# tum-vision/dvo_slam

Hardware: AMD Instinct MI355X
Metric: frame-pair alignments/s (640x480, 4-level pyramid) + finest-level HBM GB/s vs roofline (higher is better)
Workload: dtype f32 (Gram operands exact f16 hi + lo pairs on every level, f32 accumulate); 1 GPU; 1024 pairs (BASELINE config 4): independent 640x480 RGB-D frame pairs, seeds 0..1023, pair i on rank i mod 1, 4-level pyramid, FirstLevel=3, LastLevel=0, MaxIterationsPerLevel=100, Precision=5e-7, Mu=0; step = every rank re-ingests the raw planes of its shard from HBM (pyramids, sampling planes, point selection) and aligns it as one batch; the build of step k+1 (build stream) overlaps the match of; pairs=1024, pairs_per_gpu=1024, width=640, height=480, lanes=1 lane

## Files before the change

dvo_slam_amd/csrc/capi.hip:

```cpp
#include <hip/hip_runtime.h>
#ifdef DVO_WITH_ROCTX
#include <rocprofiler-sdk-roctx/roctx.h>
#endif
#include <xmmintrin.h>

#include <algorithm>
#include <functional>
#include <climits>
#include <cstddef>
#include <cmath>
#include <cstdio>
#include <atomic>
#include <chrono>
#include <thread>
#include <condition_variable>
#include <cstdlib>
#include <cstring>
#include <mutex>
#include <string>
#include <vector>

#include "../../include/dvo_hip.h"
#include "device_types.h"
#include "batch_policy.h"
#include "colour.h"
#include "launch.h"
#include "pose_graph.h"
#include "ref_order.h"
#include "selection.h"

using namespace dvo_hip;

namespace {

std::string g_create_error;

std::atomic<unsigned long long> g_free_epoch{1};

struct DevBuf {
  void* p = nullptr;
  size_t bytes = 0;
  hipError_t reserve(size_t n) {
    if (n <= bytes) return hipSuccess;
    if (p) {
      (void)hipFree(p);
      g_free_epoch.fetch_add(1, std::memory_order_relaxed);
    }
    p = nullptr;
    bytes = 0;
    hipError_t e = hipMalloc(&p, n);
    if (e == hipSuccess) bytes = n;
    return e;
  }
  void release() {
    if (p) {
      (void)hipFree(p);
      g_free_epoch.fetch_add(1, std::memory_order_relaxed);
    }
    p = nullptr;
    bytes = 0;
  }
  template <typename T> T* as() const { return static_cast<T*>(p); }
};

struct PinnedBuf {
  void* p = nullptr;
  size_t bytes = 0;
  hipError_t reserve(size_t n) {
    if (n <= bytes) return hipSuccess;
    release();
    hipError_t e = hipHostMalloc(&p, n, hipHostMallocCoherent | hipHostMallocMapped);
    if (e == hipSuccess) bytes = n;
    else p = nullptr;
    return e;
  }
  void release() {
    if (p) (void)hipHostFree(p);
    p = nullptr;
    bytes = 0;
  }
  template <typename T> T* as() const { return static_cast<T*>(p); }
};

struct CameraGeom {
  int w0 = 0, h0 = 0, levels = 0;
  float K0[4] = {0, 0, 0, 0};
  int w[kMaxLevels], h[kMaxLevels];
  float K[kMaxLevels][4];
  float* tx[kMaxLevels];
  float* ty[kMaxLevels];
  DevBuf tables;
};

struct FrameLevel {
  int w = 0, h = 0;
  float* I = nullptr;
  float* Z = nullptr;
  float4* A = nullptr;
  float2* B = nullptr;
  float2* R = nullptr;
  float2* C = nullptr;
  int cur_have = 0;
  bool selected = false;
  bool q3 = false;
  bool explicit_sel = false;
  float ithr = 0, dthr = 0;
};
// ... 201 lines not shown
  int cap_levels = 0, cap_iters = 0;
  hipEvent_t after = nullptr;
  int rc = DVO_HIP_OK;
};


struct dvo_hip_context {
  std::recursive_mutex mutex;
  int device = 0;
  hipStream_t stream = nullptr;
  std::string err;
  int opt_rows_per_wave = 0;
  int opt_iters_per_sync = 0;
  struct MatchRequest {
    dvo_hip_frame* reference; dvo_hip_frame* current; const dvo_hip_config* cfg; dvo_hip_result* result;
    dvo_hip_level_stats* levels; int cap_levels; dvo_hip_iteration_stats* iters; int cap_iters;
    std::atomic<int> state{0};
    int rc = 0;
  };
  std::mutex rendezvous_mutex;
  MatchRequest* rendezvous_waiting = nullptr;
  dvo_hip_frame* rendezvous_busy_current = nullptr;
  int rendezvous_expect = 0;
  int opt_rendezvous = 1;
  long long rendezvous_pairs = 0;
  long long f16_range_repeats = 0;
  long long strip_ingests = 0;
  long long colour_ingests = 0;
  long long f32_ingests = 0;
  long long lens_ingests = 0;
  long long depth_registrations = 0;
  long long map_inserts = 0, map_points = 0, map_dropped = 0;
  long long map_removes = 0, map_rehashes = 0;
  int opt_graph_resident = 0;
  long long graph_resident_solves = 0;
  long long map_renders = 0;
  struct DeferredIngest {
    std::vector<dvo_hip_frame*> frames;
    std::vector<const void*> planes, depth;
    int format = 0;
    size_t pitch = 0;
    int depth_format = 0;
    size_t depth_pitch = 0;
    float depth_scale;
    int role;
    dvo_hip_config cfg;
    bool keep_raw_copy;
  };
  std::vector<DeferredIngest> deferred;
  int opt_defer_ingest = 0;
  int opt_defer_ingest_pixels = 0;
  int opt_keep_raw_copy = 1;
  long long deferred_ingests = 0;
  int opt_build_workgroups = 0;
  int opt_stream_policy = 1;
  int opt_tail_speculation = 0;
  int opt_solver_waves = 0;
  int opt_ll_blocks = 0;
  int opt_compact_residuals = 1;
  int opt_gram_lo_parts = 1;
  int opt_min_workgroups = 0;
  int opt_condition_number = 0;
  int opt_fused_ll_pixels = 0;
  float last_sel_ithr = 0.0f, last_sel_dthr = 0.0f;
  int f32_gram_hold = 0;
  long long warmup_wait_us = 0;
  int opt_variant = 8;
  int opt_resident = -1;
  int opt_resident_rows = 0;
  int opt_resident_group = 0;
  int resident_timeouts = 0;
  long long resident_launches = 0;
  long long resident_levels = 0;
  long long host_ns[4] = {0, 0, 0, 0};
  long long host_batches = 0;
  std::chrono::steady_clock::time_point batch_entry;
  int opt_resident_flags = 0;
  int opt_sweep_tail = 0;
  long long tail_steps = 0;
  int opt_overlap_tails = 0;
  int opt_overlap_fraction = 8;
  int opt_tail_lists = 0;
  long long listed_steps = 0;
  long long overlapped_tails = 0;
  long long overlapped_steps = 0;
  long long tail_drains = 0;
  long long tail_wait_ns = 0;
  int opt_batch_groups = 0;
  bool is_twin = false;
  std::vector<GroupWorker*> group_workers;
  hipEvent_t roles_ready = nullptr;
  long long grouped_batches = 0;
  int opt_small_sweep = 0;
  int opt_small_tiles = 0;
  int opt_coarse = 0;
  int opt_coarse_pixels = 0;
  int opt_coarse_wgs = 0;
  long long coarse_launches = 0, coarse_levels = 0;
  int opt_deterministic = 0;
  int opt_ref_compat = 0;
  int opt_ref_order = 0;
  long long ref_order_passes = 0;
  DevBuf ref_order_planes;
  DevBuf rcp_table;
  int rcp_shift = 0;
  int rcp_packed = 0;
  int opt_resident_cooperative = 0;
  int compute_units = 0;
  std::vector<CameraGeom*> cameras;
  struct PooledBlock { void* p; size_t bytes; };
  std::vector<PooledBlock> frame_pool;
  size_t frame_pool_bytes = 0;
  static constexpr size_t kFramePoolMaxBytes = size_t(1) << 30;
  static constexpr size_t kFramePoolMaxBlocks = 64;
  Workspace ws[1];
  DevBuf misc, role_tbl_cur, role_tbl_ref, prep_tbl_cur, prep_tbl_ref;
  DevBuf sel_tbl_main, sel_tbl_build;
  unsigned long long sel_visits = 0;
  DevBuf lens_tbl;
  DevBuf graph_jobs, graph_outs;
  DevBuf rig_tbl;
  DevBuf colour_tbl, colour_stage;
  DevBuf map_tbl, map_stage;
  DevBuf render_tbl, render_zbuf, render_planes;
  hipEvent_t render_done = nullptr;
  static const int kTableSlots = 4;
  DevBuf build_tbl[kTableSlots];
  DevBuf* build_tbl_cur = nullptr;
  unsigned build_tbl_next = 0;
  PinnedRing tables;
  std::vector<dvo_hip_frame*> build_tbl_frames;
  hipStream_t build_stream = nullptr;
  static const int kBuildRing = 16;
  hipEvent_t build_events[kBuildRing] = {};
  unsigned long long build_seq = 0;
  unsigned long long main_waited_seq = 0;
  hipStream_t upload_stream = nullptr;
  hipEvent_t upload_done = nullptr;
  static const int kUploadRing = 3;
  DevBuf upload_buf[kUploadRing];
  unsigned long long upload_buf_seq[kUploadRing] = {};
  unsigned upload_next = 0;
  unsigned long long upload_waited_seq = 0;
};

namespace {
int flush_deferred(dvo_hip_context* ctx);
}

#define DVO_FLUSH_DEFERRED(ctx)                                     \
  do {                                                              \
    if ((ctx) && !(ctx)->deferred.empty()) {                        \
      const int rc_deferred__ = flush_deferred(ctx);                \
      if (rc_deferred__ != DVO_HIP_OK) return rc_deferred__;        \
    }                                                               \
  } while (0)

#define DVO_LOCK(ctx)                                               \
  std::unique_lock<std::recursive_mutex> guard;                     \
  if (ctx) guard = std::unique_lock<std::recursive_mutex>((ctx)->mutex)
#define DVO_ENTER(ctx) \
  DVO_LOCK(ctx);       \
  DVO_FLUSH_DEFERRED(ctx)

namespace {

// ... 914 lines not shown
```

dvo_slam_amd/csrc/capi_groups.inc:

```
void mirror_options(const dvo_hip_context* from, dvo_hip_context* to) {
#define DVO_MIRROR(f) to->f = from->f
  DVO_MIRROR(opt_rows_per_wave); DVO_MIRROR(opt_iters_per_sync); DVO_MIRROR(opt_tail_speculation); DVO_MIRROR(opt_solver_waves);
  DVO_MIRROR(opt_ll_blocks); DVO_MIRROR(opt_compact_residuals); DVO_MIRROR(opt_gram_lo_parts); DVO_MIRROR(opt_min_workgroups);
  DVO_MIRROR(opt_condition_number); DVO_MIRROR(opt_fused_ll_pixels); DVO_MIRROR(opt_variant); DVO_MIRROR(opt_resident);
  DVO_MIRROR(opt_resident_rows); DVO_MIRROR(opt_resident_group); DVO_MIRROR(opt_resident_flags); DVO_MIRROR(opt_resident_cooperative);
  DVO_MIRROR(opt_sweep_tail); DVO_MIRROR(opt_coarse); DVO_MIRROR(opt_coarse_pixels); DVO_MIRROR(opt_coarse_wgs);
  DVO_MIRROR(opt_deterministic); DVO_MIRROR(opt_ref_order); DVO_MIRROR(opt_small_sweep); DVO_MIRROR(opt_small_tiles); DVO_MIRROR(compute_units);
  DVO_MIRROR(opt_overlap_tails); DVO_MIRROR(opt_overlap_fraction); DVO_MIRROR(opt_tail_lists); DVO_MIRROR(opt_defer_ingest_pixels);
#undef DVO_MIRROR
}

void group_worker_main(GroupWorker* gw) {
  (void)hipSetDevice(gw->twin->device);
  for (;;) {
    std::unique_lock<std::mutex> lock(gw->m);
    gw->cv.wait(lock, [&] { return gw->has_job || gw->quit; });
    if (gw->quit) return;
    gw->has_job = false;
    lock.unlock();
    dvo_hip_context* t = gw->twin;
    t->batch_entry = std::chrono::steady_clock::now();
    int rc = DVO_HIP_OK;
    if (hipStreamWaitEvent(t->stream, gw->after, 0) != hipSuccess) {
      t->err = "match: a pair group could not wait for the batch's role planes";
      rc = DVO_HIP_ERR_HIP;
    }
    if (rc == DVO_HIP_OK) {
      rc = run_batch(t, gw->n, gw->refs, gw->curs, gw->cfg, gw->results, gw->levels, gw->cap_levels, gw->iters, gw->cap_iters);
      if (rc != DVO_HIP_OK) t->err = t->ws[0].err;
    }
    lock.lock();
    gw->rc = rc;
    gw->done = true;
    lock.unlock();
    gw->cv.notify_all();
  }
}

int batch_groups_of(const dvo_hip_context* ctx, int n) {
  if (ctx->is_twin || ctx->opt_ref_compat || ctx->opt_deterministic || ctx->opt_ref_order) return 1;
  return ctx->opt_batch_groups > 1 ? std::min(ctx->opt_batch_groups, std::max(1, n / 64)) : 1;
}

int ensure_group_workers(dvo_hip_context* ctx, int groups) {
  while (int(ctx->group_workers.size()) < groups - 1) {
    dvo_hip_context* twin = nullptr;
    const int rc = dvo_hip_context_create(ctx->device, &twin);
    if (rc != DVO_HIP_OK) return fail(ctx, rc, "match: could not create a pair group's context");
    twin->is_twin = true;
    GroupWorker* gw = new GroupWorker();
    gw->twin = twin;
    gw->thread = std::thread(group_worker_main, gw);
    ctx->group_workers.push_back(gw);
  }
  if (!ctx->roles_ready) DVO_HIP_TRY(ctx, hipEventCreateWithFlags(&ctx->roles_ready, hipEventDisableTiming));
  return DVO_HIP_OK;
}

void destroy_group_workers(dvo_hip_context* ctx) {
  for (GroupWorker* gw : ctx->group_workers) {
    {
      std::lock_guard<std::mutex> lock(gw->m);
      gw->quit = true;
    }
    gw->cv.notify_all();
    if (gw->thread.joinable()) gw->thread.join();
    dvo_hip_context_destroy(gw->twin);
    delete gw;
  }
  ctx->group_workers.clear();
  if (ctx->roles_ready) (void)hipEventDestroy(ctx->roles_ready);
  ctx->roles_ready = nullptr;
}

int run_batch_grouped(dvo_hip_context* ctx, int groups, int n, dvo_hip_frame* const* refs, dvo_hip_frame* const* curs, const dvo_hip_config* cfg,
                      dvo_hip_result* results, dvo_hip_level_stats* levels, int cap_levels, dvo_hip_iteration_stats* iters, int cap_iters) {
  int rc = ensure_group_workers(ctx, groups);
  if (rc != DVO_HIP_OK) return rc;
  DVO_HIP_TRY(ctx, hipEventRecord(ctx->roles_ready, ctx->stream));
  const int base = n / groups, extra = n % groups;
  const int n0 = base + (extra > 0 ? 1 : 0);
  int at = n0;
  for (int g = 1; g < groups; ++g) {
    GroupWorker* gw = ctx->group_workers[g - 1];
    const int m = base + (g < extra ? 1 : 0);
    mirror_options(ctx, gw->twin);
    {
      std::lock_guard<std::mutex> lock(gw->m);
      gw->n = m;
      gw->refs = refs + at; gw->curs = curs + at; gw->cfg = cfg; gw->results = results + at;
      gw->levels = levels && cap_levels > 0 ? levels + size_t(at) * cap_levels : nullptr;
// ... 27 lines not shown
```

dvo_slam_amd/csrc/capi_options.inc:

```
int dvo_hip_get_counter(dvo_hip_context* ctx, const char* key, long long* value) {
  if (!ctx || !key || !value) return DVO_HIP_ERR_INVALID;
  std::unique_lock<std::recursive_mutex> guard(ctx->mutex);
  if (std::strcmp(key, "resident_launches") == 0) *value = ctx->resident_launches;
  else if (std::strcmp(key, "resident_levels") == 0) *value = ctx->resident_levels;
  else if (std::strcmp(key, "resident_timeouts") == 0) *value = ctx->resident_timeouts;
  else if (std::strcmp(key, "grouped_batches") == 0) *value = ctx->grouped_batches;
  else if (std::strcmp(key, "compute_units") == 0) *value = BatchPolicy(ctx->compute_units).cus;
  else if (std::strcmp(key, "defer_ingest_max_pairs") == 0) *value = BatchPolicy(ctx->compute_units).defer_ingest_max_pairs();
  else if (std::strcmp(key, "background_build_workgroups") == 0) *value = BatchPolicy(ctx->compute_units).background_build_workgroups();
  else if (std::strcmp(key, "tail_steps") == 0) {
    *value = ctx->tail_steps;
    for (const GroupWorker* gw : ctx->group_workers) *value += gw->twin->tail_steps;
  }
  else if (std::strcmp(key, "overlapped_tails") == 0) *value = ctx->overlapped_tails;
  else if (std::strcmp(key, "overlapped_steps") == 0) *value = ctx->overlapped_steps;
  else if (std::strcmp(key, "listed_steps") == 0) *value = ctx->listed_steps;
  else if (std::strcmp(key, "tail_drains") == 0) *value = ctx->tail_drains;
  else if (std::strcmp(key, "tail_wait_us") == 0) *value = ctx->tail_wait_ns / 1000;
  else if (std::strcmp(key, "ref_order_passes") == 0) *value = ctx->ref_order_passes;
  else if (std::strcmp(key, "coarse_launches") == 0) *value = ctx->coarse_launches;
  else if (std::strcmp(key, "coarse_levels") == 0) *value = ctx->coarse_levels;
  else if (std::strcmp(key, "window_fallbacks") == 0) {
    unsigned long long v = 0;
    if (ctx->ws[0].win_fallbacks.p) {
      DVO_HIP_TRY(ctx, hipStreamSynchronize(ctx->stream));
      DVO_HIP_TRY(ctx, hipMemcpy(&v, ctx->ws[0].win_fallbacks.p, sizeof(v), hipMemcpyDeviceToHost));
    }
    *value = (long long)v;
  }
  else if (std::strcmp(key, "strip_ingests") == 0) *value = ctx->strip_ingests;
  else if (std::strcmp(key, "colour_ingests") == 0) *value = ctx->colour_ingests;
  else if (std::strcmp(key, "f32_ingests") == 0) *value = ctx->f32_ingests;
  else if (std::strcmp(key, "lens_ingests") == 0) *value = ctx->lens_ingests;
  else if (std::strcmp(key, "depth_registrations") == 0) *value = ctx->depth_registrations;
  else if (std::strcmp(key, "depth_rig_table_bytes") == 0) *value = (long long)ctx->rig_tbl.bytes;
  else if (std::strcmp(key, "map_inserts") == 0) *value = ctx->map_inserts;
  else if (std::strcmp(key, "map_removes") == 0) *value = ctx->map_removes;
  else if (std::strcmp(key, "map_rehashes") == 0) *value = ctx->map_rehashes;
  else if (std::strcmp(key, "map_renders") == 0) *value = ctx->map_renders;
  else if (std::strcmp(key, "map_points") == 0) *value = ctx->map_points;
  else if (std::strcmp(key, "map_dropped") == 0) *value = ctx->map_dropped;
  else if (std::strcmp(key, "graph_resident_solves") == 0) *value = ctx->graph_resident_solves;
  else if (std::strcmp(key, "warmup_wait_us") == 0) *value = ctx->warmup_wait_us;
  else if (std::strcmp(key, "rendezvous_pairs") == 0) {
    std::lock_guard<std::mutex> lock(ctx->rendezvous_mutex);
    *value = ctx->rendezvous_pairs;
  }
  else if (std::strcmp(key, "f16_range_repeats") == 0) *value = ctx->f16_range_repeats;
  else if (std::strcmp(key, "table_uploads_skipped") == 0) *value = ctx->tables.skipped;
  else if (std::strcmp(key, "deferred_ingests") == 0) *value = ctx->deferred_ingests;
  else if (std::strcmp(key, "host_batches") == 0) *value = ctx->host_batches;
  else if (std::strcmp(key, "host_ns_prepare") == 0) *value = ctx->host_ns[0];
  else if (std::strcmp(key, "host_ns_enqueue") == 0) *value = ctx->host_ns[1];
  else if (std::strcmp(key, "host_ns_wait") == 0) *value = ctx->host_ns[2];
  else if (std::strcmp(key, "host_ns_finish") == 0) *value = ctx->host_ns[3];
  else return fail(ctx, DVO_HIP_ERR_INVALID, "unknown counter");
  return DVO_HIP_OK;
}

int dvo_hip_set_option(dvo_hip_context* ctx, const char* key, int value) {
  DVO_LOCK(ctx);
  if (!ctx || !key) return DVO_HIP_ERR_INVALID;
  if (std::strcmp(key, "rows_per_wave") == 0) {
    if (value != 0 && value != 1 && value != 2 && value != 4 && value != 8 && value != 16)
      return fail(ctx, DVO_HIP_ERR_INVALID, "rows_per_wave must be 0,1,2,4,8,16");
    ctx->opt_rows_per_wave = value;
    return DVO_HIP_OK;
  }
  if (std::strcmp(key, "iters_per_sync") == 0) {
    if (value < 0) return fail(ctx, DVO_HIP_ERR_INVALID, "iters_per_sync must be >= 0");
    ctx->opt_iters_per_sync = value;
    return DVO_HIP_OK;
  }
  if (std::strcmp(key, "variant") == 0) {
    if (value != 0 && (value < 5 || value > 9))
      return fail(ctx, DVO_HIP_ERR_INVALID, "variant must be 0 (all-VALU schedule), 5 (matrix-core schedule), 6 or 7 (current-frame window staged in LDS, residuals bit-identical to the oracle's), 8 or 9 (the same with contracted arithmetic)");
    if (ctx->opt_ref_order && value != 7 && value != 8) return fail(ctx, DVO_HIP_ERR_INVALID, "ref_order runs under variant 7 or 8");
    ctx->opt_variant = value;
    ctx->f32_gram_hold = 0;
    return DVO_HIP_OK;
  }
  if (std::strcmp(key, "rendezvous") == 0) {
    if (value != 0 && value != 1) return fail(ctx, DVO_HIP_ERR_INVALID, "rendezvous must be 0 or 1");
    ctx->opt_rendezvous = value;
    return DVO_HIP_OK;
  }
  if (std::strcmp(key, "ref_order") == 0) {
    if (value != 0 && value != 1) return fail(ctx, DVO_HIP_ERR_INVALID, "ref_order must be 0 or 1");
    if (value && ctx->opt_variant != 7 && ctx->opt_variant != 8) return fail(ctx, DVO_HIP_ERR_INVALID, "ref_order runs under variant 7 or 8");
    ctx->opt_ref_order = value;
    return DVO_HIP_OK;
  }
  if (std::strcmp(key, "deterministic") == 0) {
    if (value != 0 && value != 1) return fail(ctx, DVO_HIP_ERR_INVALID, "deterministic must be 0 or 1");
    ctx->opt_deterministic = value;
    return DVO_HIP_OK;
  }
  if (std::strcmp(key, "ref_compat") == 0) {
    if (value < 0 || value > 2) return fail(ctx, DVO_HIP_ERR_INVALID, "ref_compat must be 0, 1 or 2 (2: as 1, the table read through memory by every sweep)");
    if (value && !ctx->rcp_table.p) {
      const int rc = build_rcp_table(ctx);
      if (rc != DVO_HIP_OK) return rc;
    }
    ctx->opt_ref_compat = value;
    return DVO_HIP_OK;
  }
  if (std::strcmp(key, "resident") == 0) {
    if (value < -1 || value > 1) return fail(ctx, DVO_HIP_ERR_INVALID, "resident must be -1 (automatic), 0 (off) or 1 (every level)");
    ctx->opt_resident = value;
    return DVO_HIP_OK;
  }
  if (std::strcmp(key, "small_sweep") == 0) {
    if (value != 0 && value != 1) return fail(ctx, DVO_HIP_ERR_INVALID, "small_sweep must be 0 or 1");
    ctx->opt_small_sweep = value;
    return DVO_HIP_OK;
  }
  if (std::strcmp(key, "small_tiles") == 0) {
    if (value < 0 || value > 32) return fail(ctx, DVO_HIP_ERR_INVALID, "small_tiles must be 0 (by batch size) .. 32");
    ctx->opt_small_tiles = value;
    return DVO_HIP_OK;
  }
  if (std::strcmp(key, "batch_groups") == 0) {
    if (value < 0 || value > 4) return fail(ctx, DVO_HIP_ERR_INVALID, "batch_groups must be 0 or 1 (one group) .. 4");
    ctx->opt_batch_groups = value;
    return DVO_HIP_OK;
  }
  if (std::strcmp(key, "solver_occupancy") == 0) {
    if (value != 0 && value != 3) return fail(ctx, DVO_HIP_ERR_INVALID, "solver_occupancy must be 0 or 3");
    g_solver_occupancy = value;
    return DVO_HIP_OK;
  }
  if (std::strcmp(key, "sweep_tail") == 0) {
    if (value < 0 || value > 2) return fail(ctx, DVO_HIP_ERR_INVALID, "sweep_tail must be 0, 1 (the whole step in the sweep's tail) or 2 (its wide half; the serial half in a launch behind it)");
    ctx->opt_sweep_tail = value;
    return DVO_HIP_OK;
  }
  if (std::strcmp(key, "overlap_tails") == 0) {
    if (value < 0 || value > 1) return fail(ctx, DVO_HIP_ERR_INVALID, "overlap_tails must be 0 (off) or 1 (a level's stragglers finish beside the next level)");
    ctx->opt_overlap_tails = value;
    return DVO_HIP_OK;
  }
  if (std::strcmp(key, "defer_ingest_pixels") == 0) {
    if (value < 0) return fail(ctx, DVO_HIP_ERR_INVALID, "defer_ingest_pixels must be >= 0");
    ctx->opt_defer_ingest_pixels = value;
    return DVO_HIP_OK;
  }
  if (std::strcmp(key, "tail_lists") == 0) {
    if (value < 0 || value > 1) return fail(ctx, DVO_HIP_ERR_INVALID, "tail_lists must be 0 or 1 (the last steps of a costly level are launched over the list of pairs still on it)");
    ctx->opt_tail_lists = value;
    return DVO_HIP_OK;
  }
  if (std::strcmp(key, "overlap_fraction") == 0) {
    if (value < 2 || value > 64) return fail(ctx, DVO_HIP_ERR_INVALID, "overlap_fraction must be in [2, 64]: a level's tail is split off once at most 1/value of the pairs is on it");
    ctx->opt_overlap_fraction = value;
    return DVO_HIP_OK;
  }
  if (std::strcmp(key, "coarse") == 0) {
    if (value < 0 || value > 1) return fail(ctx, DVO_HIP_ERR_INVALID, "coarse must be 0 (off) or 1 (whenever the levels admit it)");
    ctx->opt_coarse = value;
    return DVO_HIP_OK;
  }
  if (std::strcmp(key, "coarse_pixels") == 0) {
    if (value < 0) return fail(ctx, DVO_HIP_ERR_INVALID, "coarse_pixels must be >= 0");
    ctx->opt_coarse_pixels = value;
    return DVO_HIP_OK;
  }
  if (std::strcmp(key, "coarse_workgroups") == 0) {
    if (value != 0 && value != 3 && value != 4) return fail(ctx, DVO_HIP_ERR_INVALID, "coarse_workgroups must be 0, 3 or 4");
    ctx->opt_coarse_wgs = value;
    return DVO_HIP_OK;
  }
  if (std::strcmp(key, "resident_flags") == 0) {
    ctx->opt_resident_flags = value;
    return DVO_HIP_OK;
  }
  if (std::strcmp(key, "resident_cooperative") == 0) {
    ctx->opt_resident_cooperative = value != 0;
    return DVO_HIP_OK;
  }
  if (std::strcmp(key, "resident_rows") == 0) {
    if (value < 0) return fail(ctx, DVO_HIP_ERR_INVALID, "resident_rows must be >= 0");
    ctx->opt_resident_rows = value;
    return DVO_HIP_OK;
  }
  if (std::strcmp(key, "resident_group") == 0) {
    if (value < 0 || value > kResidentMaxGroup || (value & (value - 1))) return fail(ctx, DVO_HIP_ERR_INVALID, "resident_group must be 0 or a power of two <= 64");
    ctx->opt_resident_group = value;
    return DVO_HIP_OK;
  }
  if (std::strcmp(key, "build_workgroups") == 0) {
    if (value < 0) return fail(ctx, DVO_HIP_ERR_INVALID, "build_workgroups must be >= 0");
    ctx->opt_build_workgroups = value;
    return DVO_HIP_OK;
  }
  if (std::strcmp(key, "tail_speculation") == 0) {
    if (value < 0) return fail(ctx, DVO_HIP_ERR_INVALID, "tail_speculation must be >= 0");
    ctx->opt_tail_speculation = value;
    return DVO_HIP_OK;
  }
  if (std::strcmp(key, "solver_waves") == 0) {
    if (value != 0 && value != 2 && value != 4) return fail(ctx, DVO_HIP_ERR_INVALID, "solver_waves must be 0, 2 or 4");
    ctx->opt_solver_waves = value;
    return DVO_HIP_OK;
  }
  if (std::strcmp(key, "ll_blocks") == 0) {
    if (value < 0 || value > kLlBlocksPerPair) return fail(ctx, DVO_HIP_ERR_INVALID, "ll_blocks must be 0..32");
    ctx->opt_ll_blocks = value;
    return DVO_HIP_OK;
  }
  if (std::strcmp(key, "gram_lo_parts") == 0) {
    if (value != 0 && value != 1) return fail(ctx, DVO_HIP_ERR_INVALID, "gram_lo_parts must be 0 or 1");
    ctx->opt_gram_lo_parts = value;
    return DVO_HIP_OK;
  }
  if (std::strcmp(key, "compact_residuals") == 0) {
    if (value != 0 && value != 1) return fail(ctx, DVO_HIP_ERR_INVALID, "compact_residuals must be 0 or 1");
    ctx->opt_compact_residuals = value;
    return DVO_HIP_OK;
  }
  if (std::strcmp(key, "min_workgroups") == 0) {
    if (value < 0) return fail(ctx, DVO_HIP_ERR_INVALID, "min_workgroups must be >= 0");
    ctx->opt_min_workgroups = value;
    return DVO_HIP_OK;
  }
  if (std::strcmp(key, "condition_number") == 0) {
    if (value != 0 && value != 1) return fail(ctx, DVO_HIP_ERR_INVALID, "condition_number must be 0 or 1");
    ctx->opt_condition_number = value;
    return DVO_HIP_OK;
  }
  if (std::strcmp(key, "defer_ingest") == 0) {
    if (value != 0 && value != 1) return fail(ctx, DVO_HIP_ERR_INVALID, "defer_ingest must be 0 or 1");
    ctx->opt_defer_ingest = value;
    if (!value) DVO_FLUSH_DEFERRED(ctx);
    return DVO_HIP_OK;
// ... 30 lines not shown
```

dvo_slam_amd/csrc/capi_schedule.inc:

```
struct BatchPlan {
  int n = 0, nlev = 0, cap_levels = 0, cap_iters = 0;
  SolverParams prm;
  const CameraGeom* cam = nullptr;
  std::vector<int> rpw;
  std::vector<LevelGeom> geom;
  PairPtrs* pair_ptrs = nullptr;
  std::vector<PairPtrs> host_ptrs;
  int coarse_levels = 0;
  bool ref_order = false;
};

int validate_batch(dvo_hip_context* ctx, int n, dvo_hip_frame* const* refs, dvo_hip_frame* const* curs, const dvo_hip_config* cfg) {
  if (!ctx || n < 1 || !refs || !curs || !cfg) return fail(ctx, DVO_HIP_ERR_INVALID, "match: null argument");
  if (cfg->first_level < cfg->last_level || cfg->last_level < 0 || cfg->first_level >= kMaxLevels)
    return fail(ctx, DVO_HIP_ERR_INVALID, "match: need 0 <= last_level <= first_level < DVO_HIP_MAX_LEVELS");
  if (cfg->max_iterations_per_level < 1) return fail(ctx, DVO_HIP_ERR_INVALID, "match: max_iterations_per_level < 1");
  const int need_levels = cfg->first_level + 1;
  const CameraGeom* cam = refs[0] ? refs[0]->cam : nullptr;
  for (int i = 0; i < n; ++i) {
    if (!refs[i] || !curs[i]) return fail(ctx, DVO_HIP_ERR_INVALID, "match: null frame");
    if (refs[i]->levels < need_levels || curs[i]->levels < need_levels)
      return fail(ctx, DVO_HIP_ERR_INVALID, "match: frame pyramid has fewer levels than first_level + 1");
    if (refs[i]->cam != cam || curs[i]->cam != cam)
      return fail(ctx, DVO_HIP_ERR_INVALID, "match: all frames of a batch must share size and intrinsics");
// ... 403 lines not shown
  args.levels = w.lvl_stats.as<dvo_hip_level_stats>();
  args.iters = w.it_stats.as<dvo_hip_iteration_stats>();
  args.T_init = w.t_init.as<double>();
  args.partials = w.partials.as<float>();
  args.scratch = w.scratch.as<float2>();
  args.fallback_count = w.win_fallbacks.as<unsigned long long>();
  args.f16_range_flag = w.f16_range_flag;
  args.prm = bp.prm;
  args.n_pairs = bp.n;
  args.first_level = cfg->first_level;
  args.last_level = cfg->first_level - bp.coarse_levels + 1;
  for (int l = args.last_level; l <= args.first_level; ++l) {
    args.max_tiles = std::max(args.max_tiles, bp.geom[l].tiles_x * bp.geom[l].tiles_y);
    args.max_entries = std::max(args.max_entries, residual_entries(bp.geom[l]));
  }
  args.results = args.last_level == cfg->last_level ? w.results.as<dvo_hip_result>() : nullptr;
  ctx->coarse_launches += 1;
  ctx->coarse_levels += bp.coarse_levels;
  DVO_WS_TRY(w, launch_match_coarse(w.stream, args, ctx->opt_coarse_wgs == 3 ? 3 : 4));
  return DVO_HIP_OK;
}

std::mutex g_rare_path_mutex;

constexpr int kF32GramHoldBatches = 32;

hipEvent_t g_trace_ev[2] = {nullptr, nullptr};

int run_batch(dvo_hip_context* ctx, int n, dvo_hip_frame* const* refs, dvo_hip_frame* const* curs, const dvo_hip_config* cfg,
              dvo_hip_result* results, dvo_hip_level_stats* levels, int cap_levels, dvo_hip_iteration_stats* iters, int cap_iters) {
  Workspace& w = ctx->ws[0];
  hipStream_t s = w.stream;
  static const double trace_slow_ms = std::getenv("DVO_HIP_TRACE_SLOW") ? std::atof(std::getenv("DVO_HIP_TRACE_SLOW")) : 0.0;
  double mark_ms[5] = {0, 0, 0, 0, 0};
  auto mark = [&](int k) { if (trace_slow_ms > 0.0) mark_ms[k] = std::chrono::duration<double, std::milli>(std::chrono::steady_clock::now() - ctx->batch_entry).count(); };
  mark(0);
  if (trace_slow_ms > 0.0) {
    if (!g_trace_ev[0]) { (void)hipEventCreate(&g_trace_ev[0]); (void)hipEventCreate(&g_trace_ev[1]); }
    (void)hipEventRecord(g_trace_ev[0], s);
  }
  struct VariantScope {
    dvo_hip_context* c; int keep;
    ~VariantScope() { c->opt_variant = keep; }
  } variant_scope{ctx, ctx->opt_variant};
  BatchPlan bp;
  make_plan(ctx, refs[0]->cam, cfg, n, bp);
  const BatchPolicy policy(ctx->compute_units);
  const ResidentPlan rp = plan_paths(ctx, cfg, bp, window_taps_missing(ctx, cfg, n, curs));
  const bool tables_inline = rp.direct && n <= kResidentInline;
  int rc = prepare_buffers(w, cfg, refs, curs, bp, !tables_inline);
  if (rc != DVO_HIP_OK) return rc;
  mark(1);

  std::vector<double> tinit(size_t(n) * 16);
  for (int i = 0; i < n; ++i) std::memcpy(&tinit[size_t(i) * 16], results[i].transformation, 16 * sizeof(double));
  if (!tables_inline) DVO_WS_TRY(w, w.tables->upload(s, w.t_init.p, tinit.data(), tinit.size() * sizeof(double)));
  const size_t main_steps = size_t(bp.cap_iters) + 8 + kResidentErrorWords;
  bool overlap_batch = ctx->opt_overlap_tails != 0 && !ctx->opt_ref_order && !policy.level_hand_over(n) && ctx->opt_sweep_tail == 0 && rp.levels == 0 && bp.coarse_levels == 0 &&
                       cfg->first_level > cfg->last_level;
  for (int l = cfg->last_level; l <= cfg->first_level; ++l)
    overlap_batch = overlap_batch && sweep_takes_pair_list(ctx->opt_variant, bp.rpw[l], bp.geom[l]);
  const size_t tail_steps_cap = overlap_batch ? size_t(bp.cap_iters) + 12 * size_t(bp.nlev) + 8 : 0;
  const size_t n_steps = main_steps + tail_steps_cap;
  if (overlap_batch) {
    size_t t_tiles = 1, t_entries = 0;
    for (int l = cfg->last_level; l <= cfg->first_level; ++l) {
      t_tiles = std::max(t_tiles, size_t(bp.geom[l].tiles_x) * bp.geom[l].tiles_y);
      t_entries = std::max(t_entries, residual_entries(bp.geom[l]));
    }
    DVO_WS_TRY(w, w.tail_partials.reserve(size_t(n) * t_tiles * kAccStride * sizeof(float)));
    DVO_WS_TRY(w, w.tail_scratch.reserve(size_t(n) * t_entries * sizeof(float2)));
    DVO_WS_TRY(w, w.tail_flags.reserve(align_up(size_t(n), 256)));
    DVO_WS_TRY(w, w.tail_ll.reserve(size_t(n) * kLlBlocksPerPair * sizeof(double)));

    DVO_WS_TRY(w, w.counters.reserve(n_steps * sizeof(unsigned long long) + align_up(size_t(n) * sizeof(int), 8)));
    if (!w.tail_stream) {
      int prio_least = 0, prio_greatest = 0;
      DVO_WS_TRY(w, hipDeviceGetStreamPriorityRange(&prio_least, &prio_greatest));
      DVO_WS_TRY(w, hipStreamCreateWithPriority(&w.tail_stream, hipStreamNonBlocking, prio_greatest));
      DVO_WS_TRY(w, hipEventCreateWithFlags(&w.tail_split, hipEventDisableTiming));
      DVO_WS_TRY(w, hipEventCreateWithFlags(&w.tail_end, hipEventDisableTiming));
    }
  }
  if (overlap_batch || ctx->opt_tail_lists) DVO_WS_TRY(w, w.tail_list.reserve(3 * align_up(size_t(n), 64) * sizeof(int)));
  if (w.needs_drain) {
    if (w.tail_stream) DVO_WS_TRY(w, hipStreamSynchronize(w.tail_stream));
    DVO_WS_TRY(w, sync_stream(s));
    if (w.f16_range_flag) std::memset(w.f16_range_flag, 0, w.f16_range_words * sizeof(int));
  }
  w.needs_drain = true;
  mark(2);
  rc = ensure_host_status(w, n_steps);
  if (rc != DVO_HIP_OK) return rc;
  mark(3);
  w.resident_error_word = int(w.resident_launch_counter++ % kResidentErrorWords);
  if (rp.direct) {
    w.host_status[w.resident_error_word] = 0;
  } else {
    if (trace_slow_ms > 0.0) (void)hipEventRecord(g_trace_ev[1], s);
    if (w.device_may_lag) DVO_WS_TRY(w, sync_stream(s));
    w.device_may_lag = false;
    if (trace_slow_ms > 0.0) {
      mark(4);
      float gpu_ms = -1.0f;
      if (mark_ms[4] - mark_ms[3] > trace_slow_ms && hipEventElapsedTime(&gpu_ms, g_trace_ev[0], g_trace_ev[1]) == hipSuccess)
        std::fprintf(stderr, "dvo_hip: the stream wait took %.3f ms on the host; on the device %.3f ms passed between the batch's first and last command so far\n",
                     mark_ms[4] - mark_ms[3], gpu_ms);
    }
    std::memset(w.host_status, 0, n_steps * sizeof(int));
    DVO_WS_TRY(w, hipMemsetAsync(w.counters.p, 0, n_steps * sizeof(unsigned long long) + align_up(size_t(n) * sizeof(int), 8), s));
  }

  PairState* states = w.states.as<PairState>();
  dvo_hip_level_stats* d_levels = w.lvl_stats.as<dvo_hip_level_stats>();
  dvo_hip_iteration_stats* d_iters = w.it_stats.as<dvo_hip_iteration_stats>();
  float* partials = w.partials.as<float>();
  float2* scratch = w.scratch.as<float2>();
  double* ll_partials = w.ll_partials.as<double>();
  RefOrderPair* const ref_order = bp.ref_order ? w.ref_pairs.as<RefOrderPair>() : nullptr;
  unsigned long long* tallies = w.counters.as<unsigned long long>();
  int* arrivals = reinterpret_cast<int*>(tallies + n_steps);
  const int per_level = cfg->max_iterations_per_level;
  const int per_sync = ctx->opt_iters_per_sync > 0 ? ctx->opt_iters_per_sync : 1;
  int step = kResidentErrorWords;
  mark(4);
  if (trace_slow_ms > 0.0 && mark_ms[4] > trace_slow_ms)
    std::fprintf(stderr, "dvo_hip: slow preparation of a %d-pair batch: roles %.3f, plan + buffers + tables %.3f, initial guesses + drain %.3f, status words %.3f, "
                 "stream wait + reset %.3f ms\n", n, mark_ms[0], mark_ms[1] - mark_ms[0], mark_ms[2] - mark_ms[1], mark_ms[3] - mark_ms[2], mark_ms[4] - mark_ms[3]);
  const auto t_launch = std::chrono::steady_clock::now();
  int level_from = cfg->first_level;
  const bool want_stats = (levels && cap_levels > 0) || (iters && cap_iters > 0);
  ResidentBudget::Hold compute_units;
  if (rp.levels > 0 && rp.group > 1)
    compute_units.take(ResidentBudget::of(ctx->device), n * rp.group, ctx->compute_units > 0 ? ctx->compute_units : 256);
  if (rp.levels > 0) {
    Range range("resident");
    rc = run_resident(ctx, w, cfg, bp, rp, tinit.data(), want_stats);
    if (rc != DVO_HIP_OK) return rc;
    if (!ctx->deferred.empty()) {
      const int rc_deferred = flush_deferred(ctx);
      if (rc_deferred != DVO_HIP_OK) {
        w.err = ctx->err;
        return rc_deferred;
      }
    }
    level_from = cfg->first_level - rp.levels;
  }
  if (bp.coarse_levels > 0) {
    Range range("coarse");
    rc = run_coarse(ctx, w, cfg, bp);
    if (rc != DVO_HIP_OK) return rc;
    if (!ctx->deferred.empty()) {
      const int rc_deferred = flush_deferred(ctx);
      if (rc_deferred != DVO_HIP_OK) {
        w.err = ctx->err;
        return rc_deferred;
      }
    }
    level_from = cfg->first_level - bp.coarse_levels;
  }
  struct LevelSchedule {
    bool fused_ll = false, two_waves = false;
    int ll_blocks = 0;
  };
  auto schedule_of = [&](int level) {
    const LevelGeom& g = bp.geom[level];
    LevelSchedule ls;
// ... 53 lines not shown
        return;
      }
      const int lv = sl.level - 1;
      launch_level_begin(w.tail_stream, states, n, bp.prm, bp.geom[lv], lv, bp.pair_ptrs + size_t(lv) * n, d_levels, nullptr, lane_flags, 1, sl.level);
      sl.level = lv;
      sl.valid_from = tail_next;
      sl.last_active = -1;
      tail_enqueue(3);
      return;
    }
    if (tail_next - sl.seen < 2) tail_enqueue(2);
  };
  auto tail_shed = [&](int level, int active) -> int {
    Range range("shed");
    const int next_sel = sl.live ? sl.list_sel ^ 1 : 0;
    const int cap = std::min(n, sl.cap + active);
    launch_mark_stragglers(s, states, n, level, lane_flags, lane_list(next_sel), cap);
    DVO_WS_TRY(w, hipEventRecord(w.tail_split, s));
    DVO_WS_TRY(w, hipStreamWaitEvent(w.tail_stream, w.tail_split, 0));
    sl.cap = cap;
    sl.list_sel = next_sel;
    if (!sl.live) {
      sl.live = true;
      sl.level = level;
    }
    sl.valid_from = tail_next;
    sl.last_active = -1;
    tail_enqueue(3);
    ctx->overlapped_tails += 1;
    return DVO_HIP_OK;
  };
  auto wait_main = [&](int idx, int* active) -> int {
    if (!sl.live || sl.done) return wait_for_step(w, idx, active);
    volatile int* word = w.host_status + idx;
    const auto t0 = std::chrono::steady_clock::now();
    for (unsigned spins = 1;; ++spins) {
      const int v = *word;
      if (v & kStepDoneFlag) {
        *active = v & ~kStepDoneFlag;
        tail_service();
        return DVO_HIP_OK;
      }
      if ((spins & 0x3f) == 0) tail_service();
      if ((spins & 0xfffff) == 0) {
        const int rc_check = step_wait_check(w, t0);
        if (rc_check != DVO_HIP_OK) return rc_check;
      }
    }
  };

  for (int level = level_from; level >= cfg->last_level; --level) {
    main_level = level;
    LevelGeom g = bp.geom[level];
    if (sl.live) g.skip_flags = lane_flags;
    const PairPtrs* pp = bp.pair_ptrs + size_t(level) * n;
    static const char* const kPrep[kMaxLevels] = {"prep L0", "prep L1", "prep L2", "prep L3", "prep L4", "prep L5", "prep L6", "prep L7"};
    static const char* const kErr[kMaxLevels] = {"err L0", "err L1", "err L2", "err L3", "err L4", "err L5", "err L6", "err L7"};
    static const char* const kLinsys[kMaxLevels] = {"linsys L0", "linsys L1", "linsys L2", "linsys L3", "linsys L4", "linsys L5", "linsys L6", "linsys L7"};
    const bool hand_over = policy.level_hand_over(n);
    if (level == level_from || !hand_over) {
      Range range(kPrep[level]);
      launch_level_begin(s, states, n, bp.prm, g, level, pp, d_levels, level == cfg->first_level ? w.t_init.as<double>() : nullptr,
                         sl.live ? lane_flags : nullptr, 0);
    }
    NextLevel next;
    std::memset(&next, 0, sizeof(next));
    if (hand_over && level > cfg->last_level) {
      const LevelGeom& gn = bp.geom[level - 1];
      next.valid = 1;
      next.level = level - 1;
      next.fx = gn.fx; next.fy = gn.fy; next.ox = gn.ox; next.oy = gn.oy;
      next.pairs = bp.pair_ptrs + size_t(level - 1) * n;
    } else if (hand_over) {
      next.results = w.results.as<dvo_hip_result>();
    }
    const LevelSchedule schedule = schedule_of(level);
    const bool fused_ll = schedule.fused_ll;
    const int ll_blocks = schedule.ll_blocks;
    const bool solver_two_waves = schedule.two_waves;
    const bool tail = ctx->opt_sweep_tail != 0 && fused_ll && sweep_has_tail(ctx->opt_variant, bp.rpw[level], g);
    double* pair_sums = tail && ctx->opt_sweep_tail == 2 ? w.pair_sums.as<double>() : nullptr;
    LevelGeom g_run = g;
    int n_run = n;
    auto enqueue_chunk = [&](int count) {
      for (int c = 0; c < count; ++c, ++step) {
        if (tail) {
          Range range(kErr[level]);
          const SolverStepArgs a = make_solver_step_args(states, n, bp.prm, partials, ll_partials, ll_blocks, scratch, d_levels, d_iters, tallies + step, w.host_status + step,
                                                         cfg->first_level - level, &next, arrivals, pair_sums);
          launch_residual_reduce(s, ctx->opt_variant, bp.rpw[level], level == 0, g, pp, states, n, partials, scratch, w.win_fallbacks.as<unsigned long long>(),
                                 w.f16_range_flag, &a);
          if (pair_sums) {
            Range range2(kLinsys[level]);
            launch_solver_serial(s, n, g, a);
          }
          ctx->tail_steps += 1;
          continue;
        }
        {
          Range range(kErr[level]);
          launch_residual_reduce(s, ctx->opt_variant, bp.rpw[level], level == 0, g_run, pp, states, n_run, partials, scratch, w.win_fallbacks.as<unsigned long long>(),
                                 w.f16_range_flag);
          if (ref_order) {
            launch_ref_order(s, g_run, states, n_run, scratch, w.ref_rows.as<RefOrderSeg>(), ref_order);
            ctx->ref_order_passes += 1;
          }
          if (!fused_ll) launch_loglik(s, g_run, states, n_run, partials, scratch, ll_partials, ll_blocks, ctx->opt_deterministic != 0, ref_order);
        }
        if (g_run.pair_list) ctx->listed_steps += 1;
        Range range(kLinsys[level]);
        launch_solver_step(s, states, n_run, bp.prm, g_run, partials, ll_partials, ll_blocks, fused_ll ? scratch : nullptr, d_levels, d_iters,
                           tallies + step, w.host_status + step, solver_two_waves, cfg->first_level - level, &next, ref_order);
      }
    };
    int enqueued = std::min(per_sync, per_level);
    enqueue_chunk(enqueued);
    const bool flush_here = ctx->opt_defer_ingest_pixels <= 0 || g.w * g.h >= ctx->opt_defer_ingest_pixels || level == cfg->last_level;
    if (!ctx->deferred.empty() && flush_here) {
      if (size_t(g.tiles_x) * g.tiles_y * size_t(n) < 65536) {
        const int lead = std::min(policy.deferred_ingest_lead(n) * per_sync, per_level - enqueued);
        if (lead > 0) {
          enqueue_chunk(lead);
          enqueued += lead;
        }
      }
      const int rc_deferred = flush_deferred(ctx);
      if (rc_deferred != DVO_HIP_OK) {
        w.err = ctx->err;
        return rc_deferred;
      }
    }
    int watched = step - 1;
    const bool list_tails = ctx->opt_tail_lists != 0 && !bp.ref_order && !tail && !hand_over && sweep_takes_pair_list(ctx->opt_variant, bp.rpw[level], g);
    const bool may_shed = overlap_batch && level > cfg->last_level && !tail && sweep_takes_pair_list(ctx->opt_variant, bp.rpw[level], g);
    const bool empty_step_is_costly = size_t(g.tiles_x) * g.tiles_y * size_t(n) >= (ctx->opt_tail_speculation >= 2 ? size_t(ctx->opt_tail_speculation) : kCostlyEmptyStepWorkgroups) && ctx->opt_tail_speculation != 1;
    int last_active = n;
    for (;;) {
      const bool hold = empty_step_is_costly && last_active * 8 <= n;
      int more = hold ? 0 : std::min(per_sync, per_level - enqueued);
      if (more > 0) {
        enqueue_chunk(more);
        enqueued += more;
      }
      int active = 0;
      rc = wait_main(watched, &active);
      if (rc != DVO_HIP_OK) return rc;
      last_active = active;
      if (may_shed && active > 0 && size_t(active) * size_t(ctx->opt_overlap_fraction) <= size_t(n)) {
        rc = tail_shed(level, active);
        if (rc != DVO_HIP_OK) return rc;
        break;
      }
      if (hold && active > 0) {
        if (list_tails && !g_run.pair_list) {
          int* const own_list = w.tail_list.as<int>() + 2 * align_up(size_t(n), 64);
          launch_mark_stragglers(s, states, n, level, sl.live ? lane_flags : nullptr, own_list, active, true);
          g_run.pair_list = own_list;
          n_run = active;
        }
        more = std::min(per_sync, per_level - enqueued);
        if (more > 0) {
          enqueue_chunk(more);
          enqueued += more;
        }
      }
      if (active == 0 || more <= 0) break;
      watched = step - 1;
    }
    if (hand_over && step - 1 <= watched) {
      Range range(kLinsys[level]);
      launch_solver_step(s, states, n, bp.prm, g, partials, ll_partials, ll_blocks, nullptr, d_levels, d_iters, tallies + step, w.host_status + step,
                         solver_two_waves, cfg->first_level - level, &next, ref_order);
      ++step;
    }
  }

  if (sl.live) {
    main_level = cfg->last_level - 1;
    const auto t_wait = std::chrono::steady_clock::now();
    tail_service();
    while (!sl.done) {
      if (tail_next == 0 || size_t(tail_next) >= tail_steps_cap) {
        w.err = "match: the slow lane of the batch ran out of steps";
        return DVO_HIP_ERR_HIP;
      }
      int unused = 0;
      rc = wait_for_step(w, int(main_steps) + tail_next - 1, &unused);
      if (rc != DVO_HIP_OK) return rc;
      tail_service();
    }
    ctx->tail_drains += 1;
    ctx->tail_wait_ns += std::chrono::duration_cast<std::chrono::nanoseconds>(std::chrono::steady_clock::now() - t_wait).count();
    DVO_WS_TRY(w, hipStreamWaitEvent(s, w.tail_end, 0));
  }
  const bool resident_used = rp.levels > 0;
  std::vector<dvo_hip_level_stats> hl;
  std::vector<dvo_hip_iteration_stats> hi;
  const dvo_hip_level_stats* hl_src = nullptr;
  const dvo_hip_iteration_stats* hi_src = nullptr;
  std::chrono::steady_clock::time_point t_enqueued, t_done;
  if (rp.direct) {
    t_enqueued = std::chrono::steady_clock::now();
    rc = wait_for_direct(w, n);
    w.device_may_lag = true;
    if (rc != DVO_HIP_OK) return rc;
    t_done = std::chrono::steady_clock::now();
    if (w.host_status[w.resident_error_word] == 0) {
      std::memcpy(results, w.direct_results.p, size_t(n) * sizeof(dvo_hip_result));
      if (levels && cap_levels > 0) hl_src = w.direct_levels.as<dvo_hip_level_stats>();
      if (iters && cap_iters > 0) hi_src = w.direct_iters.as<dvo_hip_iteration_stats>();
    } else {
      DVO_WS_TRY(w, sync_stream(s));
    }
  } else {
    if (level_from >= cfg->last_level && policy.finish_launch(n)) launch_finish(s, states, n, bp.prm, d_levels, d_iters, w.results.as<dvo_hip_result>());
    DVO_WS_TRY(w, hipMemcpyAsync(results, w.results.p, size_t(n) * sizeof(dvo_hip_result), hipMemcpyDeviceToHost, s));
    if (levels && cap_levels > 0) {
      hl.resize(size_t(n) * bp.cap_levels);
      DVO_WS_TRY(w, hipMemcpyAsync(hl.data(), d_levels, hl.size() * sizeof(dvo_hip_level_stats), hipMemcpyDeviceToHost, s));
      hl_src = hl.data();
    }
    if (iters && cap_iters > 0) {
      hi.resize(size_t(n) * bp.cap_iters);
      DVO_WS_TRY(w, hipMemcpyAsync(hi.data(), d_iters, hi.size() * sizeof(dvo_hip_iteration_stats), hipMemcpyDeviceToHost, s));
      hi_src = hi.data();
    }
    t_enqueued = std::chrono::steady_clock::now();
    DVO_WS_TRY(w, sync_stream(s));
    DVO_WS_TRY(w, hipGetLastError());
    t_done = std::chrono::steady_clock::now();
  }
  if (resident_used && w.host_status[w.resident_error_word] != 0) {
    w.resident_sequence = 0xffffffffu;
    ctx->resident_timeouts += 1;
    if (ctx->resident_timeouts >= 3) ctx->opt_resident_group = 1;
    for (int i = 0; i < n; ++i) std::memcpy(results[i].transformation, &tinit[size_t(i) * 16], 16 * sizeof(double));
    const int keep = ctx->opt_resident;
    ctx->opt_resident = 0;
    w.needs_drain = true;
    rc = ensure_batch_roles(ctx, n, refs, curs, cfg);
    if (rc == DVO_HIP_OK) rc = run_batch(ctx, n, refs, curs, cfg, results, levels, cap_levels, iters, cap_iters);
    ctx->opt_resident = keep;
    return rc;
  }
  std::vector<int> out_of_range;
  if (ctx->opt_variant >= 7)
    for (int i = 0; i < n; ++i)
      if (static_cast<volatile int*>(w.f16_range_flag)[i] != 0) {
        static_cast<volatile int*>(w.f16_range_flag)[i] = 0;
        out_of_range.push_back(i);
      }
// ... 70 lines not shown
```

Before: 93990 alignments/s.

## Forecast per-level active pair counts from past batches to hold or list costly steps

Adds a per-configuration history of how many pairs stayed active after each step on a level. On costly levels it uses that history to stop speculatively enqueuing steps, or to switch to a straggler pair list, before the observed active count has dropped. The aim is to avoid enqueuing GPU steps that find no work or little work. If a forecast turns out wrong, its history is dropped, and such a miss can add a pipeline bubble while the host waits to enqueue more steps. The per-step forecasts use the highest active count seen across the last few batches.

```diff
diff --git a/dvo_slam_amd/csrc/capi.hip b/dvo_slam_amd/csrc/capi.hip
--- a/dvo_slam_amd/csrc/capi.hip
+++ b/dvo_slam_amd/csrc/capi.hip
@@ -23,6 +23,7 @@
 #include "../../include/dvo_hip.h"
 #include "device_types.h"
 #include "batch_policy.h"
+#include "step_forecast.h"
 #include "colour.h"
 #include "launch.h"
 #include "pose_graph.h"
@@ -390,6 +391,11 @@
   int opt_overlap_fraction = 8;
   int opt_tail_lists = 0;
   long long listed_steps = 0;
+  int opt_step_forecast = 1;
+  StepForecast step_forecast;
+  long long forecast_held_steps = 0, forecast_listed_steps = 0;
+  long long forecast_bubbles = 0;
+  long long empty_costly_steps = 0;
   long long overlapped_tails = 0;
   long long overlapped_steps = 0;
   long long tail_drains = 0;
diff --git a/dvo_slam_amd/csrc/capi_groups.inc b/dvo_slam_amd/csrc/capi_groups.inc
--- a/dvo_slam_amd/csrc/capi_groups.inc
+++ b/dvo_slam_amd/csrc/capi_groups.inc
@@ -7,6 +7,7 @@
   DVO_MIRROR(opt_sweep_tail); DVO_MIRROR(opt_coarse); DVO_MIRROR(opt_coarse_pixels); DVO_MIRROR(opt_coarse_wgs);
   DVO_MIRROR(opt_deterministic); DVO_MIRROR(opt_ref_order); DVO_MIRROR(opt_small_sweep); DVO_MIRROR(opt_small_tiles); DVO_MIRROR(compute_units);
   DVO_MIRROR(opt_overlap_tails); DVO_MIRROR(opt_overlap_fraction); DVO_MIRROR(opt_tail_lists); DVO_MIRROR(opt_defer_ingest_pixels);
+  DVO_MIRROR(opt_step_forecast);
 #undef DVO_MIRROR
 }
 
diff --git a/dvo_slam_amd/csrc/capi_options.inc b/dvo_slam_amd/csrc/capi_options.inc
--- a/dvo_slam_amd/csrc/capi_options.inc
+++ b/dvo_slam_amd/csrc/capi_options.inc
@@ -15,6 +15,10 @@
   else if (std::strcmp(key, "overlapped_tails") == 0) *value = ctx->overlapped_tails;
   else if (std::strcmp(key, "overlapped_steps") == 0) *value = ctx->overlapped_steps;
   else if (std::strcmp(key, "listed_steps") == 0) *value = ctx->listed_steps;
+  else if (std::strcmp(key, "forecast_held_steps") == 0) *value = ctx->forecast_held_steps;
+  else if (std::strcmp(key, "forecast_listed_steps") == 0) *value = ctx->forecast_listed_steps;
+  else if (std::strcmp(key, "forecast_bubbles") == 0) *value = ctx->forecast_bubbles;
+  else if (std::strcmp(key, "empty_costly_steps") == 0) *value = ctx->empty_costly_steps;
   else if (std::strcmp(key, "tail_drains") == 0) *value = ctx->tail_drains;
   else if (std::strcmp(key, "tail_wait_us") == 0) *value = ctx->tail_wait_ns / 1000;
   else if (std::strcmp(key, "ref_order_passes") == 0) *value = ctx->ref_order_passes;
@@ -150,6 +154,11 @@
     ctx->opt_tail_lists = value;
     return DVO_HIP_OK;
   }
+  if (std::strcmp(key, "step_forecast") == 0) {
+    if (value < 0 || value > 1) return fail(ctx, DVO_HIP_ERR_INVALID, "step_forecast must be 0 or 1 (a costly level's steps are held back or listed by what the last batches of the same kind needed)");
+    ctx->opt_step_forecast = value;
+    return DVO_HIP_OK;
+  }
   if (std::strcmp(key, "overlap_fraction") == 0) {
     if (value < 2 || value > 64) return fail(ctx, DVO_HIP_ERR_INVALID, "overlap_fraction must be in [2, 64]: a level's tail is split off once at most 1/value of the pairs is on it");
     ctx->opt_overlap_fraction = value;
diff --git a/dvo_slam_amd/csrc/capi_schedule.inc b/dvo_slam_amd/csrc/capi_schedule.inc
--- a/dvo_slam_amd/csrc/capi_schedule.inc
+++ b/dvo_slam_amd/csrc/capi_schedule.inc
@@ -509,7 +509,7 @@
       DVO_WS_TRY(w, hipEventCreateWithFlags(&w.tail_end, hipEventDisableTiming));
     }
   }
-  if (overlap_batch || ctx->opt_tail_lists) DVO_WS_TRY(w, w.tail_list.reserve(3 * align_up(size_t(n), 64) * sizeof(int)));
+  if (overlap_batch || ctx->opt_tail_lists || ctx->opt_step_forecast) DVO_WS_TRY(w, w.tail_list.reserve(3 * align_up(size_t(n), 64) * sizeof(int)));
   if (w.needs_drain) {
     if (w.tail_stream) DVO_WS_TRY(w, hipStreamSynchronize(w.tail_stream));
     DVO_WS_TRY(w, sync_stream(s));
@@ -729,6 +729,7 @@
     double* pair_sums = tail && ctx->opt_sweep_tail == 2 ? w.pair_sums.as<double>() : nullptr;
     LevelGeom g_run = g;
     int n_run = n;
+    bool listed_by_forecast = false;
     auto enqueue_chunk = [&](int count) {
       for (int c = 0; c < count; ++c, ++step) {
         if (tail) {
@@ -755,6 +756,7 @@
           if (!fused_ll) launch_loglik(s, g_run, states, n_run, partials, scratch, ll_partials, ll_blocks, ctx->opt_deterministic != 0, ref_order);
         }
         if (g_run.pair_list) ctx->listed_steps += 1;
+        if (g_run.pair_list && listed_by_forecast) ctx->forecast_listed_steps += 1;
         Range range(kLinsys[level]);
         launch_solver_step(s, states, n_run, bp.prm, g_run, partials, ll_partials, ll_blocks, fused_ll ? scratch : nullptr, d_levels, d_iters,
                            tallies + step, w.host_status + step, solver_two_waves, cfg->first_level - level, &next, ref_order);
@@ -778,13 +780,27 @@
       }
     }
     int watched = step - 1;
-    const bool list_tails = ctx->opt_tail_lists != 0 && !bp.ref_order && !tail && !hand_over && sweep_takes_pair_list(ctx->opt_variant, bp.rpw[level], g);
+    const bool can_list = !bp.ref_order && !tail && !hand_over && sweep_takes_pair_list(ctx->opt_variant, bp.rpw[level], g);
+    const bool list_tails = ctx->opt_tail_lists != 0 && can_list;
     const bool may_shed = overlap_batch && level > cfg->last_level && !tail && sweep_takes_pair_list(ctx->opt_variant, bp.rpw[level], g);
-    const bool empty_step_is_costly = size_t(g.tiles_x) * g.tiles_y * size_t(n) >= (ctx->opt_tail_speculation >= 2 ? size_t(ctx->opt_tail_speculation) : kCostlyEmptyStepWorkgroups) && ctx->opt_tail_speculation != 1;
+    const bool step_is_costly = size_t(g.tiles_x) * g.tiles_y * size_t(n) >= (ctx->opt_tail_speculation >= 2 ? size_t(ctx->opt_tail_speculation) : kCostlyEmptyStepWorkgroups);
+    const bool empty_step_is_costly = step_is_costly && ctx->opt_tail_speculation != 1;
+    ForecastKey forecast_key;
+    forecast_key.w = g.w; forecast_key.h = g.h; forecast_key.n = n;
+    forecast_key.first_level = cfg->first_level; forecast_key.last_level = cfg->last_level; forecast_key.max_iterations = per_level;
+    forecast_key.precision = cfg->precision; forecast_key.mu = cfg->mu; forecast_key.use_initial_estimate = cfg->use_initial_estimate ? 1 : 0;
+    forecast_key.schedule = per_sync * 16 + ctx->opt_variant;
+    LevelForecast forecast(ctx->opt_step_forecast != 0 && empty_step_is_costly && !bp.ref_order && !tail && !overlap_batch ? &ctx->step_forecast : nullptr, forecast_key);
     int last_active = n;
     for (;;) {
-      const bool hold = empty_step_is_costly && last_active * 8 <= n;
-      int more = hold ? 0 : std::min(per_sync, per_level - enqueued);
+      const int polled = enqueued;
+      const int room = std::min(per_sync, per_level - enqueued);
+      const bool hold_observed = empty_step_is_costly && last_active * 8 <= n;
+      const LevelForecast::Advice advice = forecast.before_poll(polled);
+      const bool hold = hold_observed || advice != LevelForecast::kEnqueue;
+      const bool held_by_forecast = hold && !hold_observed && room > 0;
+      if (held_by_forecast) ctx->forecast_held_steps += 1;
+      int more = hold ? 0 : room;
       if (more > 0) {
         enqueue_chunk(more);
         enqueued += more;
@@ -793,17 +809,21 @@
       rc = wait_main(watched, &active);
       if (rc != DVO_HIP_OK) return rc;
       last_active = active;
+      if (active == 0 && more > 0 && step_is_costly && !g_run.pair_list) ctx->empty_costly_steps += more;
+      if (forecast.after_poll(polled, active, held_by_forecast)) ctx->forecast_bubbles += 1;
       if (may_shed && active > 0 && size_t(active) * size_t(ctx->opt_overlap_fraction) <= size_t(n)) {
         rc = tail_shed(level, active);
         if (rc != DVO_HIP_OK) return rc;
         break;
       }
       if (hold && active > 0) {
-        if (list_tails && !g_run.pair_list) {
+        const bool list_forecast = can_list && advice != LevelForecast::kEnqueue && size_t(active) * 8 <= size_t(n);
+        if (((list_tails && hold_observed) || list_forecast) && !g_run.pair_list) {
           int* const own_list = w.tail_list.as<int>() + 2 * align_up(size_t(n), 64);
           launch_mark_stragglers(s, states, n, level, sl.live ? lane_flags : nullptr, own_list, active, true);
           g_run.pair_list = own_list;
           n_run = active;
+          listed_by_forecast = !(list_tails && hold_observed);
         }
         more = std::min(per_sync, per_level - enqueued);
         if (more > 0) {
@@ -814,6 +834,7 @@
       if (active == 0 || more <= 0) break;
       watched = step - 1;
     }
+    forecast.finish();
     if (hand_over && step - 1 <= watched) {
       Range range(kLinsys[level]);
       launch_solver_step(s, states, n, bp.prm, g, partials, ll_partials, ll_blocks, nullptr, d_levels, d_iters, tallies + step, w.host_status + step,
diff --git a/dvo_slam_amd/csrc/step_forecast.h b/dvo_slam_amd/csrc/step_forecast.h
--- /dev/null
+++ b/dvo_slam_amd/csrc/step_forecast.h
@@ -0,0 +1,147 @@
+#pragma once
+
+#include <vector>
+
+namespace dvo_hip {
+
+struct ForecastKey {
+  int w = 0, h = 0, n = 0;
+  int first_level = 0, last_level = 0, max_iterations = 0;
+  double precision = 0.0, mu = 0.0;
+  int use_initial_estimate = 0;
+  int schedule = 0;
+  bool operator==(const ForecastKey& o) const {
+    return w == o.w && h == o.h && n == o.n && first_level == o.first_level && last_level == o.last_level && max_iterations == o.max_iterations &&
+           precision == o.precision && mu == o.mu && use_initial_estimate == o.use_initial_estimate && schedule == o.schedule;
+  }
+};
+
+class StepForecast {
+ public:
+  static constexpr int kBatches = 4;
+  static constexpr int kMinBatches = 2;
+  static constexpr int kMaxEntries = 32;
+
+  struct Entry {
+    ForecastKey key;
+    std::vector<int> active[kBatches];
+    int batches = 0, next = 0;
+    unsigned long long used = 0;
+
+    int predicted_active_after(int steps) const {
+      if (batches < kMinBatches || steps < 1) return -1;
+      int most = 0;
+      for (int b = 0; b < batches; ++b) {
+        const std::vector<int>& a = active[b];
+        if (a.empty()) return -1;
+        int v;
+        if (size_t(steps) <= a.size()) v = a[size_t(steps) - 1];
+        else if (a.back() == 0) v = 0;
+        else return -1;
+        if (v > most) most = v;
+      }
+      return most;
+    }
+    void remember(const std::vector<int>& counts) {
+      active[next] = counts;
+      next = (next + 1) % kBatches;
+      if (batches < kBatches) batches += 1;
+    }
+    void drop() {
+      for (std::vector<int>& a : active) a.clear();
+      batches = next = 0;
+    }
+  };
+
+  const Entry* find(const ForecastKey& key) const {
+    for (const Entry& e : entries_)
+      if (e.key == key) return &e;
+    return nullptr;
+  }
+  int predicted_active_after(const ForecastKey& key, int steps) const {
+    const Entry* e = find(key);
+    return e ? e->predicted_active_after(steps) : -1;
+  }
+  void remember(const ForecastKey& key, const std::vector<int>& counts, bool contradicted = false) {
+    Entry* e = const_cast<Entry*>(find(key));
+    if (!e) {
+      if (int(entries_.size()) < kMaxEntries) {
+        entries_.emplace_back();
+        e = &entries_.back();
+      } else {
+        e = &entries_[0];
+        for (Entry& c : entries_)
+          if (c.used < e->used) e = &c;
+        e->drop();
+      }
+      e->key = key;
+    }
+    if (contradicted) e->drop();
+    e->remember(counts);
+    e->used = ++clock_;
+  }
+  int size() const { return int(entries_.size()); }
+
+ private:
+  std::vector<Entry> entries_;
+  unsigned long long clock_ = 0;
+};
+
+class LevelForecast {
+ public:
+  enum Advice {
+    kEnqueue,
+    kHoldEnded,
+    kHoldFew,
+  };
+
+  LevelForecast(StepForecast* table, const ForecastKey& key) : table_(table), key_(key), n_(key.n) {
+    entry_ = table_ ? table_->find(key_) : nullptr;
+    live_ = entry_ != nullptr && entry_->batches >= StepForecast::kMinBatches;
+  }
+
+  bool live() const { return live_; }
+
+  Advice before_poll(int steps) {
+    advice_ = kEnqueue;
+    if (!live_) return advice_;
+    const int p = entry_->predicted_active_after(steps);
+    if (p < 0 || size_t(p) * 8 > size_t(n_)) return advice_;
+    advice_ = p == 0 ? kHoldEnded : kHoldFew;
+    return advice_;
+  }
+
+  bool after_poll(int steps, int active, bool held) {
+    if (!table_) return false;
+    if (steps >= 1) {
+      const int carried = seen_.empty() ? n_ : seen_.back();
+      if (seen_.size() < size_t(steps)) seen_.resize(size_t(steps), carried);
+      seen_[size_t(steps) - 1] = active;
+    }
+    if (!live_ || !held || advice_ == kEnqueue) return false;
+    const bool miss = advice_ == kHoldEnded ? active > 0 : size_t(active) * 8 > size_t(n_);
+    if (miss) {
+      live_ = false;
+      contradicted_ = true;
+    }
+    return miss;
+  }
+
+  void finish() {
+    if (table_ && !seen_.empty()) table_->remember(key_, seen_, contradicted_);
+    table_ = nullptr;
+    entry_ = nullptr;
+    live_ = false;
+  }
+
+ private:
+  StepForecast* table_;
+  ForecastKey key_;
+  int n_;
+  const StepForecast::Entry* entry_ = nullptr;
+  bool live_ = false, contradicted_ = false;
+  Advice advice_ = kEnqueue;
+  std::vector<int> seen_;
+};
+
+}
```

New measurement: 96330 alignments/s (median of 6 runs). 1.02x the previous value.
